# Harshs27/uGLAD

Hardware: AMD Instinct MI355X
Metric: GLAD unroll-steps/sec (batch D×D Θ-updates), M=1024 D=128 L=30 (higher is better)
Workload: dtype f32; 1 GPU; multi-task M=1024/GPU D=128 L=30 fp32 (BASELINE config 3; global batch 1024); pass=training step: forward + loss + backward + gradient exchange + Adam, sqrt_mode=ns10, parallelism=batch-sharded x1

## Files before the change

uglad_amd/csrc/cell_bwd.h:

```cpp
template <int NT>
__global__ __launch_bounds__(kThreads) void UGLAD_CELL_BWD_NAME(
    const float* __restrict__ Gnext, const float* __restrict__ S, const float* __restrict__ Zin,
    const float* __restrict__ half, const float* __restrict__ U, const float* __restrict__ beta,
    const float* __restrict__ lam_ptr, const float* __restrict__ params, float* __restrict__ Gout,
    float* __restrict__ grad_rho_partial, float* __restrict__ glam_partial, float* __restrict__ gws, int D, int mode,
#if UGLAD_CELL_BWD_GS
    int gs, int k_count, int lam_stride, float* __restrict__ gS) {
#else
    int gs, int k_count, int lam_stride) {
#endif
  constexpr int DP = NT * 32, LD = DP + 1;
  UGLAD_BIG_BUFFERS(sX, DP * LD, sY, DP * LD, gws)
  __shared__ float s_beta[DP], s_r[DP];
  __shared__ __attribute__((aligned(16))) float s_a0[DP], s_aN[DP];
  __shared__ float s_red[8];
  __shared__ float s_g[kWaves][kNRho + 1];
  const int tid = threadIdx.x, lane = tid & 63, w = tid >> 6;
  const size_t base = (size_t)blockIdx.x * D * D;
  const float* Sm = S + base;
  const float* Gm = Gnext + base;
  float* Go = Gout + base;
  const int grp = blockIdx.x / gs;
  params += (size_t)grp * kNParam;
  const size_t step_mdd = (size_t)gridDim.x * D * D, step_md = (size_t)gridDim.x * D;
  constexpr bool kPackA = NT <= 7;
  float g[kNRho];
  [[maybe_unused]] v2f g2[kNRho];
#pragma unroll
  for (int q = 0; q < kNRho; ++q) g[q] = 0.f, g2[q] = splat2(0.f);
  constexpr int kMaxQ = ((DP / 2) * (DP + 1) + kThreads - 1) / kThreads;
  constexpr bool kPre = DP <= 128;
  constexpr int kQ = kPre ? kMaxQ : 8;
  constexpr int kIShift = kPre ? 8 : 16, kJMask = (1 << kIShift) - 1;
  const int D1 = D + 1, total = ((D + 1) / 2) * D1;
  const int sp = kThreads / D1, sc = kThreads - sp * D1;
  auto entry = [&](int e, int p, int c) -> int {
    if (e >= total) return -1;
    if (c < D - p) return (p << kIShift) | (p + c);
    const int i = D - 1 - p;
    return (i == p) ? -1 : ((i << kIShift) | (i + (c - (D - p))));
  };
  auto advance = [&](int& p, int& c) {
    c += sc;
    p += sp;
    if (c >= D1) {
      c -= D1;
      ++p;
    }
  };
  __shared__ unsigned short s_ent[kPre ? kMaxQ : 1][kPre ? kThreads : 1];
  if constexpr (kPre) {
    int p = tid / D1, c = tid - p * D1;
    for (int q = 0; q < kMaxQ; ++q) {
      s_ent[q][tid] = (unsigned short)entry(tid + kThreads * q, p, c);
      advance(p, c);
    }
  }
#pragma unroll 1
  for (int s = 0; s < k_count; ++s) {
    const bool first = (s == 0), last = (s == k_count - 1);
    const int tid = opaque_v(threadIdx.x), lane = tid & 63;
    const int w = __builtin_amdgcn_readfirstlane(tid >> 6);
    const float* Zm = Zin + base - s * step_mdd;
    const float* Hm = half + base - s * step_mdd;
    const float* Um = U + base - s * step_mdd;
    const float* bm = beta + (size_t)blockIdx.x * D - s * step_md;
    const float lam = lam_ptr[(long)grp - (long)s * lam_stride];
    const float c4 = 4.0f / lam, inv_lam2 = 1.0f / (lam * lam);

    KSTAMP(0);
    constexpr int kV4 = DP * DP / 4, kC4 = DP / 4;
    constexpr bool kFull4 = kV4 % (8 * kThreads) == 0, kFull1 = (DP * DP) % (8 * kThreads) == 0;
    const bool vec16 = (D == DP) && (((reinterpret_cast<size_t>(U) | (first ? reinterpret_cast<size_t>(Gnext) : 0)) & 15) == 0);
    if (vec16) {
      if (first) {
        for (int v0 = 0; v0 < kV4; v0 += 8 * kThreads) {
          f4 u[8], gv[8];
#pragma unroll
          for (int q = 0; q < 8; ++q) {
            const int idx = v0 + q * kThreads + tid;
            const unsigned at = (kFull4 || idx < kV4) ? 16u * idx : 0u;
            u[q] = load_at<f4>(Um, at);
            gv[q] = load_at<f4>(Gm, at);
          }
#pragma unroll
          for (int q = 0; q < 8; ++q) {
            const int idx = v0 + q * kThreads + tid;
            if (kFull4 || idx < kV4) {
              const int i = idx / kC4, k = 4 * (idx - i * kC4);
              sX[i * LD + k] = u[q].x, sX[i * LD + k + 1] = u[q].y, sX[i * LD + k + 2] = u[q].z, sX[i * LD + k + 3] = u[q].w;
              sY[i * LD + k] = gv[q].x, sY[i * LD + k + 1] = gv[q].y, sY[i * LD + k + 2] = gv[q].z, sY[i * LD + k + 3] = gv[q].w;
            }
          }
        }
      } else {
        for (int v0 = 0; v0 < kV4; v0 += 8 * kThreads) {
          f4 u[8];
#pragma unroll
          for (int q = 0; q < 8; ++q) {
            const int idx = v0 + q * kThreads + tid;
            u[q] = load_at<f4>(Um, (kFull4 || idx < kV4) ? 16u * idx : 0u);
          }
#pragma unroll
          for (int q = 0; q < 8; ++q) {
            const int idx = v0 + q * kThreads + tid;
            if (kFull4 || idx < kV4) {
              const int i = idx / kC4, k = 4 * (idx - i * kC4);
              sX[i * LD + k] = u[q].x, sX[i * LD + k + 1] = u[q].y, sX[i * LD + k + 2] = u[q].z, sX[i * LD + k + 3] = u[q].w;
            }
          }
        }
      }
    } else {
      constexpr int si = kThreads / DP, sk = kThreads - si * DP;
      int i = tid / DP, k = tid - i * DP;
      int off = i * D + k;
      const int soff = si * D + sk, wrap = D - DP;
      if (first) {
        for (int idx0 = 0; idx0 < DP * DP; idx0 += 8 * kThreads) {
          float u[8], gv[8];
          int dst[8];
          bool in[8];
#pragma unroll
          for (int q = 0; q < 8; ++q) {
            in[q] = (kFull1 || idx0 + q * kThreads + tid < DP * DP) && i < D && k < D;
            const unsigned at = in[q] ? 4u * off : 0u;
            u[q] = load_at<float>(Um, at);
            gv[q] = load_at<float>(Gm, at);
            dst[q] = i * LD + k;
            i += si, k += sk, off += soff;
            if (k >= DP) k -= DP, ++i, off += wrap;
          }
          __builtin_amdgcn_sched_barrier(0);
#pragma unroll
          for (int q = 0; q < 8; ++q) {
            if (kFull1 || idx0 + q * kThreads + tid < DP * DP) {
              sX[dst[q]] = in[q] ? u[q] : 0.f;
              sY[dst[q]] = in[q] ? gv[q] : 0.f;
            }
          }
        }
      } else {
        for (int idx0 = 0; idx0 < DP * DP; idx0 += 8 * kThreads) {
          float u[8];
          int dst[8];
          bool in[8];
#pragma unroll
          for (int q = 0; q < 8; ++q) {
            in[q] = (kFull1 || idx0 + q * kThreads + tid < DP * DP) && i < D && k < D;
            u[q] = load_at<float>(Um, in[q] ? 4u * off : 0u);
            dst[q] = i * LD + k;
            i += si, k += sk, off += soff;
            if (k >= DP) k -= DP, ++i, off += wrap;
          }
          __builtin_amdgcn_sched_barrier(0);
#pragma unroll
          for (int q = 0; q < 8; ++q) {
            if (kFull1 || idx0 + q * kThreads + tid < DP * DP) sX[dst[q]] = in[q] ? u[q] : 0.f;
          }
        }
      }
    }
    const float be_ld = load_at<float>(bm, (tid < D) ? 4u * (unsigned)tid : 0u);
    [[maybe_unused]] float hx_a[kQ], zz_a[kQ], sv_a[kQ];
    if constexpr (kPre) {
      int ea[kQ];
#pragma unroll
      for (int u = 0; u < kQ; ++u) ea[u] = (int)(short)s_ent[u][tid];
#pragma unroll
      for (int u = 0; u < kQ; ++u) {
        const unsigned at = (unsigned)opaque_v((ea[u] >= 0) ? 4 * ((ea[u] >> kIShift) * D + (ea[u] & kJMask)) : 0);
        hx_a[u] = load_at<float>(Hm, at);
        zz_a[u] = load_at<float>(Zm, at);
        sv_a[u] = load_at<float>(Sm, at);
      }
    }
    float a2 = 0.f;
    if (tid < D) {
      const float be = be_ld;
      const float al = fmaf(be, be, c4);
      a2 = al * al;
    }
    const float nrmA = sqrtf(block_sum(a2, s_red));
    float r2 = 0.f;
    if (tid < DP) {
      float be = 0.f, r = 1.f;
      if (tid < D) {
        be = be_ld;
        r = sqrt_spectrum(be, c4, nrmA, mode);
        r2 = r * r;
      }
      s_beta[tid] = be;
      s_r[tid] = r;
    }
    const float nrmR = sqrtf(block_sum(r2, s_red));
    if (mode == UGLAD_SQRT_NS10 && tid < DP) {
      float a = s_r[tid] / nrmR;
      s_a0[tid] = a;
#pragma unroll
      for (int it = 0; it < kNsIters; ++it) a = 0.5f * a * (3.f - a * a);
      s_aN[tid] = a;
    }
    __syncthreads();

    KSTAMP(1);
    using TU = Tiles<NT, true>;
    [[maybe_unused]] const int p0 = tid / D1, c0 = tid - p0 * D1;
    float gz[kQ];
    {
      [[maybe_unused]] int p = p0, c = c0;
      for (int q0 = 0; q0 < kMaxQ; q0 += kQ) {
        int pk[kQ];
        float hx[kQ], zz[kQ], gn[kQ], sv[kQ];
        if constexpr (kPre) {
#pragma unroll
          for (int u = 0; u < kQ; ++u) pk[u] = (int)(short)s_ent[u][tid];
          float gt[kQ];
#pragma unroll
          for (int u = 0; u < kQ; ++u) {
            const int i = pk[u] >> kIShift, j = pk[u] & kJMask;
            const bool in = pk[u] >= 0;
            gn[u] = sY[opaque_v(in ? i * LD + j : 0)];
            gt[u] = sY[opaque_v(in ? j * LD + i : 0)];
          }
          static_assert(kPackA || !kPre, "the tabled entries go with the packed backward");
#pragma unroll
          for (int u = 0; u < kQ; ++u) {
            const int i = pk[u] >> kIShift, j = pk[u] & kJMask;
            hx[u] = hx_a[u], zz[u] = zz_a[u], sv[u] = sv_a[u];
            gn[u] = (i == j) ? gn[u] : 0.5f * (gn[u] + gt[u]);
          }
        } else {
#pragma unroll
          for (int u = 0; u < kQ; ++u) {
            pk[u] = (q0 + u < kMaxQ) ? entry(tid + kThreads * (q0 + u), p, c) : -1;
            advance(p, c);
            const int i = pk[u] >> kIShift, j = pk[u] & kJMask;
            const bool in = pk[u] >= 0;
            hx[u] = in ? Hm[i * D + j] : 0.f;
            zz[u] = in ? Zm[i * D + j] : 0.f;
            sv[u] = in ? Sm[i * D + j] : 0.f;
            gn[u] = in ? ((i == j) ? sY[i * LD + j] : 0.5f * (sY[i * LD + j] + sY[j * LD + i])) : 0.f;
          }
        }
        constexpr int kQ2 = (kQ + 1) / 2;
        if constexpr (kPackA) {
          [[maybe_unused]] const int tid_a = opaque_v(tid);
#pragma unroll
          for (int h = 0; h < kQ2; ++h) {
            const int u0 = 2 * h, u1 = (2 * h + 1 < kQ) ? 2 * h + 1 : 2 * h;
            const bool has1 = 2 * h + 1 < kQ;
            const int e0 = kPre ? (int)(short)s_ent[kPre ? u0 : 0][kPre ? tid_a : 0] : pk[u0];
            const int e1 = kPre ? (int)(short)s_ent[kPre ? u1 : 0][kPre ? tid_a : 0] : pk[u1];
            const bool in0 = e0 >= 0, in1 = has1 && e1 >= 0;
            const int i0 = e0 >> kIShift, j0 = e0 & kJMask, i1 = e1 >> kIShift, j1 = e1 & kJMask;
            const v2f x = {hx[u0], has1 ? hx[u1] : 0.f}, s2 = {sv[u0], has1 ? sv[u1] : 0.f}, z2 = {zz[u0], has1 ? zz[u1] : 0.f};
            const v2f gn2 = {gn[u0], has1 ? gn[u1] : 0.f};
            RhoAct2 act2;
            rho_forward2(params, x, s2, z2, act2);
            const bool on0 = in0 && fabsf(x.x) > act2.rho.x, on1 = in1 && fabsf(x.y) > act2.rho.y;
            const v2f gact = {on0 ? gn2.x : 0.f, on1 ? gn2.y : 0.f};
            const v2f g_rho = {on0 ? ((x.x > 0.f) ? -gn2.x : gn2.x) : 0.f, on1 ? ((x.y > 0.f) ? -gn2.y : gn2.y) : 0.f};
            const v2f wgt = {on0 ? ((i0 == j0) ? 1.f : 2.f) : 0.f, on1 ? ((i1 == j1) ? 1.f : 2.f) : 0.f};
            v2f gx1, gx3;
            rho_backward2(params, x, s2, z2, act2, g_rho, wgt, g2, gx1, gx3);
#pragma unroll
            for (int q = 0; q < kNRho; ++q) g2[q] = opaque_f2(g2[q]);
            gx3 = opaque_f2(gx3);
#if UGLAD_CELL_BWD_GS
            if (in0) gS[base + i0 * D + j0] += rho_backward_col(params, act2.half(0), g_rho.x, 1);
            if (in1) gS[base + i1 * D + j1] += rho_backward_col(params, act2.half(1), g_rho.y, 1);
#endif
            const v2f gh = gact + gx1;
            sY[opaque_v(in0 ? i0 * LD + j0 : DP)] = gh.x;
            sY[opaque_v(in0 ? j0 * LD + i0 : DP)] = gh.x;
            if (has1) {
              sY[opaque_v(in1 ? i1 * LD + j1 : DP)] = gh.y;
              sY[opaque_v(in1 ? j1 * LD + i1 : DP)] = gh.y;
            }
            if constexpr (kPre) {
              gz[u0] = gx3.x;
              if (has1) gz[u1] = gx3.y;
            } else {
              if (in0) Go[i0 * D + j0] = gx3.x;
              if (in1) Go[i1 * D + j1] = gx3.y;
            }
          }
        } else {
#pragma unroll
        for (int h = 0; h < kQ2; ++h) {
          const int u0 = 2 * h, u1 = (2 * h + 1 < kQ) ? 2 * h + 1 : 2 * h;
          const bool has1 = 2 * h + 1 < kQ;
          if (!has1 && pk[u0] < 0) continue;
          RhoAct2 act2;
          rho_forward2(params, (v2f){hx[u0], has1 ? hx[u1] : 0.f}, (v2f){sv[u0], has1 ? sv[u1] : 0.f},
                       (v2f){zz[u0], has1 ? zz[u1] : 0.f}, act2);
#pragma unroll
          for (int c2 = 0; c2 < 2; ++c2) {
            const int u = c2 ? u1 : u0;
            if ((c2 == 0 || has1) && pk[u] >= 0) {
              const int i = pk[u] >> kIShift, j = pk[u] & kJMask;
              const RhoAct act = act2.half(c2);
              const float x = hx[u];
              const bool active = fabsf(x) > act.rho;
              const float sgn = (x > 0.f) ? 1.f : ((x < 0.f) ? -1.f : 0.f);
              const float g_rho = active ? -sgn * gn[u] : 0.f;
              float gx1, gx3;
              rho_backward(params, x, sv[u], zz[u], act, g_rho, (i == j) ? 1.f : 2.f, g, gx1, gx3);
#if UGLAD_CELL_BWD_GS
              gS[base + i * D + j] += rho_backward_col(params, act, g_rho, 1);
#endif
              const float gh = (active ? gn[u] : 0.f) + gx1;
              sY[i * LD + j] = gh;
              sY[j * LD + i] = gh;
              if (kPre) gz[u] = gx3;
              else Go[i * D + j] = gx3;
            }
          }
        }
        }
      }
    }
    __syncthreads();

    KSTAMP(2);
    using T = Tiles<NT, false>;
    {
      f32x16 acc[T::kPerWave];
      gemm_lds<NT, false, false, false>(sY, sX, acc);
      __syncthreads();
      store_tiles<NT>(sY, acc);
    }
    __syncthreads();
    KSTAMP(3);
    float glam = 0.f;
    {
      f32x16 acc[TU::kPerWave];
      gemm_lds<NT, true, false, true>(sX, sY, acc);
      __syncthreads();
      KSTAMP(4);
#pragma unroll
      for (int n = 0; n < TU::kPerWave; ++n) {
        const int t = w + kWaves * n;
        if (t < TU::kCount) {
          int I, J;
          TU::ij(t, I, J);
          const int j = J * 32 + (lane & 31);
          const float a0j = s_a0[j], aNj = s_aN[j];
          const float rj = s_r[j], bj = s_beta[j];
          const float inv_2nrmR = 1.0f / (2.f * nrmR);
#pragma unroll
          for (int e4 = 0; e4 < 4; ++e4) {
            const int i0 = I * 32 + 8 * e4 + 4 * (lane >> 5);
            float Kr[4];
            if (mode == UGLAD_SQRT_EXACT) {
#pragma unroll
              for (int r = 0; r < 4; ++r) Kr[r] = 1.0f / (s_r[i0 + r] + rj);
            } else {
              const f4 a0 = *reinterpret_cast<const f4*>(&s_a0[i0]);
              const f4 aN = *reinterpret_cast<const f4*>(&s_aN[i0]);
              Kr[0] = ns_divided_difference(a0.x, a0j, aN.x, aNj, inv_2nrmR);
              Kr[1] = ns_divided_difference(a0.y, a0j, aN.y, aNj, inv_2nrmR);
              Kr[2] = ns_divided_difference(a0.z, a0j, aN.z, aNj, inv_2nrmR);
              Kr[3] = ns_divided_difference(a0.w, a0j, aN.w, aNj, inv_2nrmR);
            }
#pragma unroll
            for (int r = 0; r < 4; ++r) {
              const int e = 4 * e4 + r, i = i0 + r;
              if (I < J || i <= j) {
                float v = 0.f;
                if (i < D && j < D) {
                  const float K = Kr[r];
                  const float cij = acc[n][e];
                  if (i == j) glam = fmaf(cij, -2.f * K * inv_lam2, glam);
                  v = cij * 0.5f * fmaf(s_beta[i] + bj, K, -1.f);
                }
                sY[i * LD + j] = v;
                sY[j * LD + i] = v;
              }
            }
          }
        }
      }
    }
    __syncthreads();
    KSTAMP(5);
    {
      f32x16 acc[T::kPerWave];
      gemm_lds<NT, false, false, false>(sX, sY, acc);
      __syncthreads();
      store_tiles<NT>(sY, acc);
    }
    __syncthreads();
    KSTAMP(6);
    {
      f32x16 acc[TU::kPerWave];
      gemm_lds<NT, false, true, true>(sY, sX, acc);
      KSTAMP(7);
      __syncthreads();
#pragma unroll
      for (int n = 0; n < TU::kPerWave; ++n) {
        const int t = w + kWaves * n;
        if (t < TU::kCount) {
          int I, J;
          TU::ij(t, I, J);
#pragma unroll
          for (int e = 0; e < 16; ++e) sY[(I * 32 + acc_row(e, lane)) * LD + J * 32 + (lane & 31)] = acc[n][e];
        }
      }
    }
    __syncthreads();
    KSTAMP(20);
    {
      [[maybe_unused]] int p = p0, c = c0;
      for (int q0 = 0; q0 < kMaxQ; q0 += kQ) {
        int pk[kQ];
        float gb[kQ], sij[kQ];
#pragma unroll
        for (int u = 0; u < kQ; ++u) {
          if constexpr (kPre) {
            pk[u] = (int)(short)s_ent[u][tid];
          } else {
            pk[u] = (q0 + u < kMaxQ) ? entry(tid + kThreads * (q0 + u), p, c) : -1;
            advance(p, c);
          }
          const bool in = pk[u] >= 0;
          const int i = pk[u] >> kIShift, j = pk[u] & kJMask;
          gb[u] = sY[in ? i * LD + j : 0];
          sij[u] = load_at<float>(Sm, in ? 4u * ((unsigned)i * (unsigned)D + (unsigned)j) : 0u);
        }
        if (kPre) {
#pragma unroll
          for (int u = 0; u < kQ; ++u) {
            const bool in = pk[u] >= 0;
            const int i = pk[u] >> kIShift, j = pk[u] & kJMask;
            const float o = gz[u] - gb[u];
            sY[in ? i * LD + j : DP] = o;
            sY[in ? j * LD + i : DP] = o;
            glam = fmaf(in ? -sij[u] * inv_lam2 * ((i == j) ? 1.f : 2.f) : 0.f, gb[u], glam);
          }
        } else {
#pragma unroll
          for (int u = 0; u < kQ; ++u) {
            if (pk[u] >= 0) {
              const int i = pk[u] >> kIShift, j = pk[u] & kJMask;
              const float o = Go[i * D + j] - gb[u];
              sY[i * LD + j] = o;
              sY[j * LD + i] = o;
              glam = fmaf(-sij[u] * inv_lam2 * ((i == j) ? 1.f : 2.f), gb[u], glam);
            }
          }
        }
#if UGLAD_CELL_BWD_GS
        {
          const float inv_lam = 1.0f / lam;
#pragma unroll
          for (int u = 0; u < kQ; ++u) {
            if (pk[u] >= 0) {
              const int i = pk[u] >> kIShift, j = pk[u] & kJMask;
              const float v = fmaf(gb[u], inv_lam, gS[base + i * D + j]);
              gS[base + i * D + j] = v;
              gS[base + j * D + i] = v;
            }
          }
        }
#endif
      }
    }
    __syncthreads();
    KSTAMP(21);
    if (last) {
      const int si = kThreads / D, sj = kThreads - si * D;
      int i = tid / D, j = tid - i * D;
      for (int idx = tid; idx < D * D; idx += kThreads) {
        Go[idx] = sY[i * LD + j];
        j += sj;
        i += si;
        if (j >= D) {
          j -= D;
          ++i;
        }
      }
    }
    KSTAMP(8);
    if (last) {
#pragma unroll
      for (int q = 0; q < kNRho; ++q) {
        if constexpr (kPackA) g[q] = g2[q].x + g2[q].y;
        const float v = wave_sum(g[q]);
        if (lane == 0) s_g[w][q] = v;
      }
    }
    {
      const float v = wave_sum(glam);
      if (lane == 0) s_g[w][kNRho] = v;
    }
    __syncthreads();
    if (tid == kNRho || (last && tid < kNRho)) {
      float v = 0.f;
#pragma unroll
      for (int ww = 0; ww < kWaves; ++ww) v += s_g[ww][tid];
      if (tid < kNRho)
        grad_rho_partial[(size_t)blockIdx.x * kNRho + tid] += v;
      else
        (glam_partial - (size_t)s * gridDim.x)[blockIdx.x] = v;
    }
    KSTAMP(9);
  }
}
```

uglad_amd/csrc/glad_device.h:

```cpp
#pragma once
#include <hip/hip_runtime.h>

namespace uglad {

#ifndef UGLAD_THREADS
#define UGLAD_THREADS 512
#endif
constexpr int kThreads = UGLAD_THREADS;
constexpr int kWaves = kThreads / 64;
constexpr int kNsIters = 10;

constexpr int P_T = 0, P_RW1 = 1, P_RB1 = 10, P_RW2 = 13, P_RB2 = 22, P_RW3 = 25, P_RB3 = 28;
constexpr int P_LW1 = 29, P_LB1 = 35, P_LW2 = 38, P_LB2 = 41;
constexpr int kNParam = 42, kNRho = 28;

typedef float f32x16 __attribute__((ext_vector_type(16)));
struct alignas(16) f4 {
  float x, y, z, w;
};

#ifdef UGLAD_SIMT_EMUL
#define UGLAD_WAVE_SYNC() simt::wave_sync_point()
#else
#define UGLAD_WAVE_SYNC() asm volatile("s_waitcnt vmcnt(0) lgkmcnt(0)" ::: "memory")
#endif

template <int CTRL, int ROW_MASK = 0xf, int BANK_MASK = 0xf>
__device__ __forceinline__ float dpp_move(float v) {
  return __int_as_float(__builtin_amdgcn_update_dpp(0, __float_as_int(v), CTRL, ROW_MASK, BANK_MASK, false));
}

__device__ __forceinline__ float lane_xor1(float v) { return dpp_move<0xb1>(v); }

__device__ __forceinline__ float sum_halves(float v) {
#ifdef UGLAD_SIMT_EMUL
  return v + __shfl_xor(v, 32);
#else
  const auto r = __builtin_amdgcn_permlane32_swap(__float_as_uint(v), __float_as_uint(v), false, false);
  return __uint_as_float(r[0]) + __uint_as_float(r[1]);
#endif
}

__device__ __forceinline__ int opaque_v(int v) {
#ifndef UGLAD_SIMT_EMUL
  asm volatile("" : "+v"(v));
#endif
  return v;
}

template <typename T>
__device__ __forceinline__ T load_at(const float* __restrict__ base, unsigned bytes) {
  return *reinterpret_cast<const T*>(reinterpret_cast<const char*>(base) + bytes);
}

__device__ __forceinline__ float opaque_f(float v) {
#ifndef UGLAD_SIMT_EMUL
  asm volatile("" : "+v"(v));
#endif
  return v;
}

__device__ __forceinline__ int lane_now() {
#ifdef UGLAD_SIMT_EMUL
  return threadIdx.x & 63;
#else
  int l;
  asm volatile("v_mbcnt_lo_u32_b32 %0, -1, 0\n\tv_mbcnt_hi_u32_b32 %0, -1, %0" : "=v"(l));
  return l;
#endif
}

__device__ __forceinline__ float bcast_lane(float v, int src) {
  return __int_as_float(__builtin_amdgcn_readlane(__float_as_int(v), src));
}

__device__ __forceinline__ float wave_sum(float v) {
  v += dpp_move<0xb1>(v);
  v += dpp_move<0x4e>(v);
  v += dpp_move<0x124>(v);
  v += dpp_move<0x128>(v);
  v += dpp_move<0x142, 0xa>(v);
  v += dpp_move<0x143, 0xc>(v);
  return __int_as_float(__builtin_amdgcn_readlane(__float_as_int(v), 63));
}

__device__ __forceinline__ float block_sum(float v, float* s_red) {
  v = wave_sum(v);
  const int lane = threadIdx.x & 63, w = threadIdx.x >> 6;
  if (lane == 0) s_red[w] = v;
  __syncthreads();
  float t = 0.f;
#pragma unroll
  for (int i = 0; i < kWaves; ++i) t += s_red[i];
  __syncthreads();
  return t;
}

__device__ __forceinline__ float exp_acc(float x) {
  const float t = x * 1.44269504f;
  float e = fmaf(x, 1.44269504f, -t);
  e = fmaf(x, 1.925963033e-8f, e);
  const float r = __builtin_amdgcn_exp2f(t);
  return fmaf(r, e * 0.69314718f, r);
}

__device__ __forceinline__ float div_acc(float a, float b) {
  float q = __builtin_amdgcn_rcpf(b);
  q = fmaf(q, fmaf(-b, q, 1.0f), q);
  return a * q;
}

__device__ __forceinline__ float sigmoidf_(float x) {
  const float t = exp_acc(-fabsf(x));
  const float s = div_acc(1.0f, 1.0f + t);
  return (x >= 0.f) ? s : 1.0f - s;
}

__device__ __forceinline__ float tanhf_(float x) {
  const float t = exp_acc(-2.0f * fabsf(x));
  return copysignf(div_acc(1.0f - t, 1.0f + t), x);
}

struct RhoAct {
  float h1[3], h2[3], rho;
};

__device__ __forceinline__ void rho_forward(const float* __restrict__ p, float x1, float x2, float x3, RhoAct& a) {
#pragma unroll
  for (int o = 0; o < 3; ++o)
    a.h1[o] = tanhf_(fmaf(p[P_RW1 + 3 * o], x1, fmaf(p[P_RW1 + 3 * o + 1], x2, fmaf(p[P_RW1 + 3 * o + 2], x3, p[P_RB1 + o]))));
#pragma unroll
  for (int o = 0; o < 3; ++o)
    a.h2[o] = tanhf_(fmaf(p[P_RW2 + 3 * o], a.h1[0], fmaf(p[P_RW2 + 3 * o + 1], a.h1[1], fmaf(p[P_RW2 + 3 * o + 2], a.h1[2], p[P_RB2 + o]))));
  a.rho = sigmoidf_(fmaf(p[P_RW3], a.h2[0], fmaf(p[P_RW3 + 1], a.h2[1], fmaf(p[P_RW3 + 2], a.h2[2], p[P_RB3]))));
}

typedef float v2f __attribute__((ext_vector_type(2)));
__device__ __forceinline__ v2f opaque_f2(v2f v) {
#ifndef UGLAD_SIMT_EMUL
  asm volatile("" : "+v"(v));
#endif
  return v;
}
__device__ __forceinline__ v2f fma2(v2f a, v2f b, v2f c) { return __builtin_elementwise_fma(a, b, c); }
__device__ __forceinline__ v2f splat2(float a) { return (v2f){a, a}; }
__device__ __forceinline__ v2f exp_acc2(v2f x) {
  const v2f t = x * 1.44269504f;
  v2f e = fma2(x, splat2(1.44269504f), -t);
  e = fma2(x, splat2(1.925963033e-8f), e);
  const v2f r = {__builtin_amdgcn_exp2f(t.x), __builtin_amdgcn_exp2f(t.y)};
  return fma2(r, e * 0.69314718f, r);
}
__device__ __forceinline__ v2f div_acc2(v2f a, v2f b) {
  v2f q = {__builtin_amdgcn_rcpf(b.x), __builtin_amdgcn_rcpf(b.y)};
  q = fma2(q, fma2(-b, q, splat2(1.0f)), q);
  return a * q;
}
__device__ __forceinline__ v2f tanh2(v2f x) {
  const v2f t = exp_acc2(-2.0f * __builtin_elementwise_abs(x));
  const v2f r = div_acc2(1.0f - t, 1.0f + t);
  return (v2f){copysignf(r.x, x.x), copysignf(r.y, x.y)};
}
__device__ __forceinline__ v2f sigmoid2(v2f x) {
  const v2f t = exp_acc2(-__builtin_elementwise_abs(x));
  const v2f s = div_acc2(splat2(1.0f), 1.0f + t);
  return (v2f){(x.x >= 0.f) ? s.x : 1.0f - s.x, (x.y >= 0.f) ? s.y : 1.0f - s.y};
}
struct RhoAct2 {
  v2f h1[3], h2[3], rho;
  __device__ __forceinline__ RhoAct half(int c) const {
    RhoAct a;
#pragma unroll
    for (int o = 0; o < 3; ++o) {
      a.h1[o] = c ? h1[o].y : h1[o].x;
      a.h2[o] = c ? h2[o].y : h2[o].x;
    }
    a.rho = c ? rho.y : rho.x;
    return a;
  }
};
__device__ __forceinline__ void rho_forward2(const float* __restrict__ p, v2f x1, v2f x2, v2f x3, RhoAct2& a) {
#pragma unroll
  for (int o = 0; o < 3; ++o)
    a.h1[o] = tanh2(fma2(splat2(p[P_RW1 + 3 * o]), x1,
                         fma2(splat2(p[P_RW1 + 3 * o + 1]), x2, fma2(splat2(p[P_RW1 + 3 * o + 2]), x3, splat2(p[P_RB1 + o])))));
#pragma unroll
  for (int o = 0; o < 3; ++o)
    a.h2[o] = tanh2(fma2(splat2(p[P_RW2 + 3 * o]), a.h1[0],
                         fma2(splat2(p[P_RW2 + 3 * o + 1]), a.h1[1], fma2(splat2(p[P_RW2 + 3 * o + 2]), a.h1[2], splat2(p[P_RB2 + o])))));
  a.rho = sigmoid2(fma2(splat2(p[P_RW3]), a.h2[0], fma2(splat2(p[P_RW3 + 1]), a.h2[1], fma2(splat2(p[P_RW3 + 2]), a.h2[2], splat2(p[P_RB3])))));
}

__device__ __forceinline__ float soft_threshold(float x, float rho) {
  const float m = fabsf(x) - rho;
  return m > 0.f ? copysignf(m, x) : 0.f;
}

__device__ __forceinline__ void rho_backward(const float* __restrict__ p, float x1, float x2, float x3, const RhoAct& a,
                                             float g_rho, float w, float* g, float& gx1, float& gx3) {
  const float go = g_rho * a.rho * (1.f - a.rho);
  const float gow = go * w;
  float ga2[3], ga1[3];
#pragma unroll
  for (int h = 0; h < 3; ++h) {
    g[(P_RW3 - 1) + h] += gow * a.h2[h];
    ga2[h] = go * p[P_RW3 + h] * (1.f - a.h2[h] * a.h2[h]);
  }
  g[P_RB3 - 1] += gow;
#pragma unroll
  for (int o = 0; o < 3; ++o) {
    const float t = ga2[o] * w;
#pragma unroll
    for (int h = 0; h < 3; ++h) g[(P_RW2 - 1) + 3 * o + h] += t * a.h1[h];
    g[(P_RB2 - 1) + o] += t;
  }
#pragma unroll
  for (int h = 0; h < 3; ++h) {
    const float s = ga2[0] * p[P_RW2 + h] + ga2[1] * p[P_RW2 + 3 + h] + ga2[2] * p[P_RW2 + 6 + h];
    ga1[h] = s * (1.f - a.h1[h] * a.h1[h]);
  }
#pragma unroll
  for (int o = 0; o < 3; ++o) {
    const float t = ga1[o] * w;
    g[(P_RW1 - 1) + 3 * o + 0] += t * x1;
    g[(P_RW1 - 1) + 3 * o + 1] += t * x2;
    g[(P_RW1 - 1) + 3 * o + 2] += t * x3;
    g[(P_RB1 - 1) + o] += t;
  }
  gx1 = ga1[0] * p[P_RW1 + 0] + ga1[1] * p[P_RW1 + 3] + ga1[2] * p[P_RW1 + 6];
  gx3 = ga1[0] * p[P_RW1 + 2] + ga1[1] * p[P_RW1 + 5] + ga1[2] * p[P_RW1 + 8];
}

__device__ __forceinline__ float rho_backward_col(const float* __restrict__ p, const RhoAct& a, float g_rho, int col) {
  const float go = g_rho * a.rho * (1.f - a.rho);
  float ga2[3], ga1[3];
#pragma unroll
  for (int h = 0; h < 3; ++h) ga2[h] = go * p[P_RW3 + h] * (1.f - a.h2[h] * a.h2[h]);
#pragma unroll
  for (int h = 0; h < 3; ++h) {
    const float s = ga2[0] * p[P_RW2 + h] + ga2[1] * p[P_RW2 + 3 + h] + ga2[2] * p[P_RW2 + 6 + h];
    ga1[h] = s * (1.f - a.h1[h] * a.h1[h]);
  }
  return ga1[0] * p[P_RW1 + col] + ga1[1] * p[P_RW1 + 3 + col] + ga1[2] * p[P_RW1 + 6 + col];
}

__device__ __forceinline__ void rho_backward2(const float* __restrict__ p, v2f x1, v2f x2, v2f x3, const RhoAct2& a, v2f g_rho,
                                              v2f w, v2f* g2, v2f& gx1, v2f& gx3) {
  const v2f go = g_rho * a.rho * (1.f - a.rho);
  const v2f gow = go * w;
  v2f ga2[3], ga1[3];
#pragma unroll
  for (int h = 0; h < 3; ++h) {
    g2[(P_RW3 - 1) + h] = fma2(gow, a.h2[h], g2[(P_RW3 - 1) + h]);
    ga2[h] = go * p[P_RW3 + h] * (1.f - a.h2[h] * a.h2[h]);
  }
  g2[P_RB3 - 1] += gow;
#pragma unroll
  for (int o = 0; o < 3; ++o) {
    const v2f t = ga2[o] * w;
#pragma unroll
    for (int h = 0; h < 3; ++h) g2[(P_RW2 - 1) + 3 * o + h] = fma2(t, a.h1[h], g2[(P_RW2 - 1) + 3 * o + h]);
    g2[(P_RB2 - 1) + o] += t;
  }
#pragma unroll
  for (int h = 0; h < 3; ++h) {
    const v2f s = (h == 0) ? fma2(ga2[2], splat2(p[P_RW2 + 6]), fma2(ga2[0], splat2(p[P_RW2]), ga2[1] * p[P_RW2 + 3]))
                           : fma2(ga2[2], splat2(p[P_RW2 + 6 + h]), fma2(ga2[1], splat2(p[P_RW2 + 3 + h]), ga2[0] * p[P_RW2 + h]));
    ga1[h] = s * (1.f - a.h1[h] * a.h1[h]);
  }
#pragma unroll
  for (int o = 0; o < 3; ++o) {
    const v2f t = ga1[o] * w;
    g2[(P_RW1 - 1) + 3 * o + 0] = fma2(t, x1, g2[(P_RW1 - 1) + 3 * o + 0]);
    g2[(P_RW1 - 1) + 3 * o + 1] = fma2(t, x2, g2[(P_RW1 - 1) + 3 * o + 1]);
    g2[(P_RW1 - 1) + 3 * o + 2] = fma2(t, x3, g2[(P_RW1 - 1) + 3 * o + 2]);
    g2[(P_RB1 - 1) + o] += t;
  }
  gx1 = fma2(ga1[2], splat2(p[P_RW1 + 6]), fma2(ga1[0], splat2(p[P_RW1 + 0]), ga1[1] * p[P_RW1 + 3]));
  gx3 = opaque_f2(ga1[2] * p[P_RW1 + 8]) + fma2(ga1[1], splat2(p[P_RW1 + 5]), ga1[0] * p[P_RW1 + 2]);
}

__device__ __forceinline__ float lambda_forward(const float* __restrict__ p, float n, float lam_prev) {
  float o = p[P_LB2];
#pragma unroll
  for (int h = 0; h < 3; ++h)
    o = fmaf(p[P_LW2 + h], tanhf(fmaf(p[P_LW1 + 2 * h], n, fmaf(p[P_LW1 + 2 * h + 1], lam_prev, p[P_LB1 + h]))), o);
  return sigmoidf_(o);
}

__device__ __forceinline__ float sqrt_spectrum(float beta, float c, float nrmA, int mode) {
  const float alpha = fmaf(beta, beta, c);
  if (mode == 0) return sqrtf(alpha);
  float y = alpha / nrmA, z = 1.f;
#pragma unroll
  for (int it = 0; it < kNsIters; ++it) {
    const float T = 0.5f * (3.f - z * y);
    y = y * T;
    z = T * z;
  }
  return y * sqrtf(nrmA);
}

__device__ __forceinline__ float ns_divided_difference(float a0_i, float a0_j, float aN_i, float aN_j, float inv_2nrmR) {
  return div_acc(aN_i + aN_j, a0_i + a0_j) * inv_2nrmR;
}

__device__ __forceinline__ float shifted_spectrum(float be, int D, float lam, int mode, double* __restrict__ s3, float& alpha,
                                                  float& cond) {
  const int tid = threadIdx.x;
  const double c4 = 4.0 / (double)lam, b = (double)be;
  const double al = b * b + c4;
  const double r_exact = sqrt(al);
  if (tid < D) {
    s3[tid] = al * al;
    s3[D + tid] = 0.5 * (r_exact - b) * b;
    s3[2 * D + tid] = b * b;
  }
  __syncthreads();
  double* part = s3 + 3 * D;
  if ((tid >> 6) == 0) {
    const double* a = s3 + ((tid >> 4) < 3 ? (tid >> 4) : 2) * D;
    double s = 0.0, mx = 0.0, mn = 1e300;
    for (int i = tid & 15; i < D; i += 16) {
      const double v = a[i];
      s += v;
      mx = v > mx ? v : mx;
      mn = v < mn ? v : mn;
    }
#pragma unroll
    for (int o = 1; o < 16; o *= 2) {
      s += __shfl_xor(s, o);
      const double mxo = __shfl_xor(mx, o), mno = __shfl_xor(mn, o);
      mx = mxo > mx ? mxo : mx;
      mn = mno < mn ? mno : mn;
    }
    if ((tid & 15) == 0 && tid < 48) part[tid >> 4] = s;
    if (tid == 32) {
      part[3] = mx;
      part[4] = mn;
    }
  }
  __syncthreads();
  const double n2 = part[0], pb = part[1], bb = part[2], b2max = part[3], b2min = part[4];
  cond = (float)((b2max + c4) / (b2min + c4));
  double a_opt = (bb > 0.0) ? -pb / bb : 0.0;
  a_opt = a_opt < 0.0 ? 0.0 : (a_opt > 1.0 ? 1.0 : a_opt);
  alpha = (float)a_opt;
  double r = r_exact;
  if (mode != 0) {
    const double nrmA = sqrt(n2);
    double y = al / nrmA, z = 1.0;
#pragma unroll
    for (int it = 0; it < kNsIters; ++it) {
      const double T = 0.5 * (3.0 - z * y);
      y = y * T;
      z = T * z;
    }
    r = y * sqrt(nrmA);
  }
  const double psi = 0.5 * (r - b) + (double)alpha * b;
  __syncthreads();
  return (tid < D) ? (float)psi : 0.f;
}

template <int DP>
__device__ __forceinline__ void pair_of(int r, int k, int& i1, int& i2) {
  constexpr int m = DP - 1;
  if (k == 0) {
    i1 = m;
    i2 = r;
  } else {
    i1 = r + k;
    if (i1 >= m) i1 -= m;
    i2 = r + m - k;
    if (i2 >= m) i2 -= m;
  }
}

template <int DP>
__device__ void jacobi_eig(float* __restrict__ A, float* __restrict__ V, float* s_t, float* s_s, float* s_h, float* s_red,
                           int* s_flag) {
  constexpr int LD = DP + 1, H = DP / 2;
  const int tid = threadIdx.x;
  float fro = 0.f;
  for (int idx = tid; idx < DP * DP; idx += kThreads) {
    const float v = A[(idx / DP) * LD + (idx % DP)];
    fro = fmaf(v, v, fro);
  }
  fro = sqrtf(block_sum(fro, s_red));
  const float thresh = 1e-8f * fro;
  for (int sweep = 0; sweep < 16; ++sweep) {
    if (tid == 0) *s_flag = 0;
    __syncthreads();
    for (int r = 0; r < DP - 1; ++r) {
      if (tid < H) {
        int p, q;
        pair_of<DP>(r, tid, p, q);
        const float apq = A[p * LD + q];
        float t = 0.f, s = 0.f, h = 0.f;
        if (fabsf(apq) > thresh) {
          const float app = A[p * LD + p], aqq = A[q * LD + q];
          const float tau = (aqq - app) / (2.f * apq);
          t = copysignf(1.f, tau) / (fabsf(tau) + sqrtf(fmaf(tau, tau, 1.f)));
          const float c = 1.f / sqrtf(fmaf(t, t, 1.f));
          s = t * c;
          h = s / (1.f + c);
          *s_flag = 1;
        }
        s_t[tid] = t;
        s_s[tid] = s;
        s_h[tid] = h;
      }
      __syncthreads();
      for (int b = tid; b < H * H; b += kThreads) {
        const int kr = b / H, kc = b - kr * H;
        int r1, r2, c1, c2;
        pair_of<DP>(r, kr, r1, r2);
        pair_of<DP>(r, kc, c1, c2);
        const float x11 = A[r1 * LD + c1], x12 = A[r1 * LD + c2], x21 = A[r2 * LD + c1], x22 = A[r2 * LD + c2];
        float z11, z12, z21, z22;
        if (kr == kc) {
          const float t = s_t[kr];
          z11 = x11 - t * x12;
          z22 = x22 + t * x12;
          z12 = (t != 0.f) ? 0.f : x12;
          z21 = (t != 0.f) ? 0.f : x21;
        } else {
          const float sr = s_s[kr], hr = s_h[kr], sc = s_s[kc], hc = s_h[kc];
          const float y11 = x11 - sr * (x21 + hr * x11), y21 = x21 + sr * (x11 - hr * x21);
          const float y12 = x12 - sr * (x22 + hr * x12), y22 = x22 + sr * (x12 - hr * x22);
          z11 = y11 - sc * (y12 + hc * y11);
          z12 = y12 + sc * (y11 - hc * y12);
          z21 = y21 - sc * (y22 + hc * y21);
          z22 = y22 + sc * (y21 - hc * y22);
        }
        A[r1 * LD + c1] = z11;
        A[r1 * LD + c2] = z12;
        A[r2 * LD + c1] = z21;
        A[r2 * LD + c2] = z22;
      }
      for (int b = tid; b < DP * H; b += kThreads) {
        const int i = b / H, kc = b - i * H;
        int c1, c2;
        pair_of<DP>(r, kc, c1, c2);
        const float sc = s_s[kc], hc = s_h[kc];
        const float v1 = V[i * LD + c1], v2 = V[i * LD + c2];
        V[i * LD + c1] = v1 - sc * (v2 + hc * v1);
        V[i * LD + c2] = v2 + sc * (v1 - hc * v2);
      }
      __syncthreads();
    }
    if (*s_flag == 0) break;
    __syncthreads();
  }
  __syncthreads();
}

template <int NT, bool UPPER>
struct Tiles {
  static constexpr int kCount = UPPER ? NT * (NT + 1) / 2 : NT * NT;
  static constexpr int kPerWave = (kCount + kWaves - 1) / kWaves;
  __device__ static __forceinline__ void ij(int t, int& I, int& J) {
    if (UPPER) {
      int i = 0, rem = t;
      while (rem >= NT - i) {
        rem -= NT - i;
        ++i;
      }
      I = i;
      J = i + rem;
    } else {
      I = t / NT;
      J = t - I * NT;
    }
  }
};

__device__ __forceinline__ int acc_row(int reg, int lane) { return (reg & 3) + 8 * (reg >> 2) + 4 * (lane >> 5); }

__device__ __forceinline__ void mfma_tile(const float* __restrict__ Ap, int a_si, int a_sk, const float* __restrict__ Bp,
                                          int b_sk, int b_sj, int K, f32x16& acc) {
  const int lane = opaque_v(threadIdx.x) & 63, li = lane & 31, kh = lane >> 5;
  const float* a = Ap + li * a_si + kh * a_sk;
  const float* b = Bp + li * b_sj + kh * b_sk;
  float a0[8], b0[8], a1[8], b1[8];
#pragma unroll
  for (int u = 0; u < 8; ++u) {
    a0[u] = a[2 * u * a_sk];
    b0[u] = b[2 * u * b_sk];
  }
  for (int k = 0; k < K; k += 16) {
    const bool more = k + 16 < K;
    const float* an = a + (more ? 16 * a_sk : 0);
    const float* bn = b + (more ? 16 * b_sk : 0);
#pragma unroll
    for (int u = 0; u < 8; ++u) {
      a1[u] = an[2 * u * a_sk];
      b1[u] = bn[2 * u * b_sk];
    }
#pragma unroll
    for (int u = 0; u < 8; ++u) acc = __builtin_amdgcn_mfma_f32_32x32x2f32(a0[u], b0[u], acc, 0, 0, 0);
#pragma unroll
    for (int u = 0; u < 8; ++u) {
      a0[u] = a1[u];
      b0[u] = b1[u];
    }
    a = an;
    b = bn;
  }
}

#if defined(UGLAD_BF16X3) && !defined(UGLAD_SIMT_EMUL)
#include "../../scripts/retired/bf16x3_tile.h"
#define UGLAD_GEMM_TILE mfma_tile_bf16x3
#else
#define UGLAD_GEMM_TILE mfma_tile
#endif

template <int NT, bool TA, bool TB, bool UPPER>
__device__ __forceinline__ void gemm_lds(const float* __restrict__ X, const float* __restrict__ Y,
                                         f32x16 (&acc)[Tiles<NT, UPPER>::kPerWave]) {
  constexpr int DP = NT * 32, LD = DP + 1;
  using T = Tiles<NT, UPPER>;
  const int w = __builtin_amdgcn_readfirstlane(opaque_v(threadIdx.x) >> 6);
#pragma unroll
  for (int n = 0; n < T::kPerWave; ++n) {
    const int t = w + kWaves * n;
#pragma unroll
    for (int e = 0; e < 16; ++e) acc[n][e] = 0.f;
    if (t < T::kCount) {
      int I, J;
      T::ij(t, I, J);
      UGLAD_GEMM_TILE(TA ? X + I * 32 : X + I * 32 * LD, TA ? 1 : LD, TA ? LD : 1, TB ? Y + J * 32 * LD : Y + J * 32,
                      TB ? 1 : LD, TB ? LD : 1, DP, acc[n]);
    }
  }
}

template <int NT>
__device__ __forceinline__ void store_tiles(float* __restrict__ Y, const f32x16 (&acc)[Tiles<NT, false>::kPerWave]) {
  constexpr int LD = NT * 32 + 1;
  using T = Tiles<NT, false>;
  const int tid = opaque_v(threadIdx.x), lane = tid & 63, w = __builtin_amdgcn_readfirstlane(tid >> 6);
#pragma unroll
  for (int n = 0; n < T::kPerWave; ++n) {
    const int t = w + kWaves * n;
    if (t < T::kCount) {
      int I, J;
      T::ij(t, I, J);
#pragma unroll
      for (int e = 0; e < 16; ++e) Y[(I * 32 + acc_row(e, lane)) * LD + J * 32 + (lane & 31)] = acc[n][e];
    }
  }
}

#ifdef UGLAD_STAMPS
__device__ unsigned long long g_cwg[4096][3];
__device__ unsigned long long g_lstamps[4][96];
__device__ unsigned long long g_kstamps[32];
#define KSTAMP(i) do { if (threadIdx.x == 0 && blockIdx.x == 0) g_kstamps[i] = __builtin_amdgcn_s_memtime(); } while (0)
#define UGLAD_STAMP(ws, i) do { if (threadIdx.x == 0 && (i) < 64) (ws).stamp[i] = __builtin_amdgcn_s_memtime(); } while (0)
#elif defined(UGLAD_PHASE_EXIT)
__device__ int g_exit_at;
#define KSTAMP(i) do { if (g_exit_at == 100 + (i)) __builtin_amdgcn_endpgm(); } while (0)
#define UGLAD_STAMP(ws, i) do { if (g_exit_at == (i)) __builtin_amdgcn_endpgm(); } while (0)
#else
#define KSTAMP(i) do {} while (0)
#define UGLAD_STAMP(ws, i) do {} while (0)
#endif

__device__ __forceinline__ void copy_out_matrix(float* __restrict__ dst, const float* __restrict__ src, int D, int LD) {
  const int tid = threadIdx.x;
  if (((D & 3) == 0) && ((reinterpret_cast<size_t>(dst) & 15) == 0)) {
    const int D4 = D >> 2;
    for (int idx = tid; idx < D * D4; idx += kThreads) {
      const int i = idx / D4, j = 4 * (idx - i * D4);
      const float* p = src + i * LD + j;
      f4 v = {p[0], p[1], p[2], p[3]};
      *reinterpret_cast<f4*>(dst + (size_t)i * D + j) = v;
    }
  } else {
    const int si = kThreads / D, sj = kThreads - si * D;
    int i = tid / D, j = tid - i * D;
    for (int idx = tid; idx < D * D; idx += kThreads) {
      dst[idx] = src[i * LD + j];
      j += sj;
      i += si;
      if (j >= D) {
        j -= D;
        ++i;
      }
    }
  }
}

template <int DP>
constexpr int kTfacFloats = (DP / 32) * 1024;
template <int DP>
constexpr int kWsPerMatrix = 3 * DP + kTfacFloats<DP>;
template <int DP>
constexpr int big_floats() {
  return 2 * ((DP * (DP + 1) + 3) & ~3);
}
#define UGLAD_BIG_BUFFERS(A, NA, B, NB, GWS)                                                                     \
  constexpr bool kGM = DP > 128;                                                                                 \
  __shared__ __attribute__((aligned(16))) float A##_lds[kGM ? 4 : (NA)];                                         \
  __shared__ __attribute__((aligned(16))) float B##_lds[kGM ? 4 : (NB)];                                         \
  float* A = kGM ? (GWS) + (size_t)gridDim.x * kWsPerMatrix<DP> + (size_t)blockIdx.x * big_floats<DP>() : A##_lds; \
  float* B = kGM ? A + big_floats<DP>() / 2 : B##_lds;

template <int DP>
__device__ __forceinline__ float* tfac_behind_flags(float* ws, int M, int m) {
  static_assert(kTfacFloats<DP> / 2 >= 4, "flags and packed T factors outgrow the T region: M + 3 <= M kTfacFloats / 2 needs kTfacFloats / 2 >= 4");
  return ws + (size_t)M * 3 * DP + ((M + 3) & ~3) + (size_t)m * (kTfacFloats<DP> / 2);
}

}
```

Measured before the change: 1.326 million unroll-steps/s.

## Split leftover upper-triangular GEMM tiles across two waves with K-split and LDS reduction

For D=128 (NT=4) the upper-triangular tile set has more tiles than waves, so a few waves ran a second full 32x32 tile while the others sat idle. This splits each extra tile's K dimension in half across two waves. Each wave writes its partial accumulator half to a shared-memory scratch buffer, and each then finishes half of the tile's rows. The aim is to balance load across waves in the two symmetric backward GEMMs, at the cost of extra LDS traffic, a scratch buffer, and more complex epilogue indexing.

Result: no change. 1.338 million unroll-steps/s (median of 6 runs) (+1.0%).

```diff
diff --git a/uglad_amd/csrc/cell_bwd.h b/uglad_amd/csrc/cell_bwd.h
--- a/uglad_amd/csrc/cell_bwd.h
+++ b/uglad_amd/csrc/cell_bwd.h
@@ -205,6 +205,7 @@
 
     KSTAMP(1);
     using TU = Tiles<NT, true>;
+    using SU = SplitUpper<NT>;
     [[maybe_unused]] const int p0 = tid / D1, c0 = tid - p0 * D1;
     float gz[kQ];
     {
@@ -336,12 +337,15 @@
     float glam = 0.f;
     {
       f32x16 acc[TU::kPerWave];
-      gemm_lds<NT, true, false, true>(sX, sY, acc);
+      if constexpr (SU::kOn) SU::template product<true, false>(sX, sY, acc);
+      else gemm_lds<NT, true, false, true>(sX, sY, acc);
       __syncthreads();
+      if constexpr (SU::kOn) SU::finish(acc);
       KSTAMP(4);
 #pragma unroll
       for (int n = 0; n < TU::kPerWave; ++n) {
-        const int t = w + kWaves * n;
+        const int t = (SU::kOn && n == 1) ? SU::tile1(w) : w + kWaves * n;
+        [[maybe_unused]] const int rofs = (SU::kOn && n == 1) ? SU::rofs1(w) : 0;
         if (t < TU::kCount) {
           int I, J;
           TU::ij(t, I, J);
@@ -351,7 +355,10 @@
           const float inv_2nrmR = 1.0f / (2.f * nrmR);
 #pragma unroll
           for (int e4 = 0; e4 < 4; ++e4) {
-            const int i0 = I * 32 + 8 * e4 + 4 * (lane >> 5);
+            if constexpr (SU::kOn) {
+              if (n == 1 && e4 >= 2) continue;
+            }
+            const int i0 = SU::kOn ? I * 32 + 8 * e4 + 4 * (lane >> 5) + rofs : I * 32 + 8 * e4 + 4 * (lane >> 5);
             float Kr[4];
             if (mode == UGLAD_SQRT_EXACT) {
 #pragma unroll
@@ -395,15 +402,24 @@
     KSTAMP(6);
     {
       f32x16 acc[TU::kPerWave];
-      gemm_lds<NT, false, true, true>(sY, sX, acc);
+      if constexpr (SU::kOn) SU::template product<false, true>(sY, sX, acc);
+      else gemm_lds<NT, false, true, true>(sY, sX, acc);
       KSTAMP(7);
       __syncthreads();
+      if constexpr (SU::kOn) SU::finish(acc);
 #pragma unroll
       for (int n = 0; n < TU::kPerWave; ++n) {
-        const int t = w + kWaves * n;
+        const int t = (SU::kOn && n == 1) ? SU::tile1(w) : w + kWaves * n;
         if (t < TU::kCount) {
           int I, J;
           TU::ij(t, I, J);
+          if constexpr (SU::kOn) {
+            if (n == 1) {
+#pragma unroll
+              for (int e = 0; e < 8; ++e) sY[(I * 32 + acc_row(e, lane) + SU::rofs1(w)) * LD + J * 32 + (lane & 31)] = acc[n][e];
+              continue;
+            }
+          }
 #pragma unroll
           for (int e = 0; e < 16; ++e) sY[(I * 32 + acc_row(e, lane)) * LD + J * 32 + (lane & 31)] = acc[n][e];
         }
diff --git a/uglad_amd/csrc/glad_device.h b/uglad_amd/csrc/glad_device.h
--- a/uglad_amd/csrc/glad_device.h
+++ b/uglad_amd/csrc/glad_device.h
@@ -554,6 +554,60 @@
   }
 }
 
+#ifndef UGLAD_SPLIT_UPPER
+#define UGLAD_SPLIT_UPPER 1
+#endif
+template <int NT>
+struct SplitUpper {
+  using T = Tiles<NT, true>;
+  static constexpr int kExtra = T::kCount - kWaves;
+  static constexpr bool kOn = UGLAD_SPLIT_UPPER && NT * 32 <= 128 && kExtra > 0 && 2 * kExtra <= 4 && T::kPerWave == 2;
+  static constexpr int kPartFloats = 2 * kExtra * 8 * 64;
+  __device__ static __forceinline__ float* part() {
+    __shared__ float s_part[kPartFloats];
+    return s_part;
+  }
+  __device__ static __forceinline__ int tile1(int w) { return (w < 2 * kExtra) ? kWaves + ((w < kExtra) ? w : w - kExtra) : T::kCount; }
+  __device__ static __forceinline__ int rofs1(int w) { return (w < kExtra) ? 0 : 16; }
+  template <bool TA, bool TB>
+  __device__ static __forceinline__ void product(const float* __restrict__ X, const float* __restrict__ Y, f32x16 (&acc)[2]) {
+    constexpr int DP = NT * 32, LD = DP + 1;
+    const int tid = opaque_v(threadIdx.x), lane = tid & 63, w = __builtin_amdgcn_readfirstlane(tid >> 6);
+#pragma unroll
+    for (int n = 0; n < 2; ++n)
+#pragma unroll
+      for (int e = 0; e < 16; ++e) acc[n][e] = 0.f;
+    {
+      int I, J;
+      T::ij(w, I, J);
+      UGLAD_GEMM_TILE(TA ? X + I * 32 : X + I * 32 * LD, TA ? 1 : LD, TA ? LD : 1, TB ? Y + J * 32 * LD : Y + J * 32, TB ? 1 : LD,
+                      TB ? LD : 1, DP, acc[0]);
+    }
+    if (w < 2 * kExtra) {
+      int I, J;
+      T::ij(tile1(w), I, J);
+      const bool owner = w < kExtra;
+      const int k0 = owner ? 0 : DP / 2;
+      const float* A = (TA ? X + I * 32 : X + I * 32 * LD) + k0 * (TA ? LD : 1);
+      const float* B = (TB ? Y + J * 32 * LD : Y + J * 32) + k0 * (TB ? 1 : LD);
+      UGLAD_GEMM_TILE(A, TA ? 1 : LD, TA ? LD : 1, B, TB ? 1 : LD, TB ? LD : 1, DP / 2, acc[1]);
+      float* mine = part() + w * 512 + lane;
+#pragma unroll
+      for (int r = 0; r < 8; ++r) mine[64 * r] = owner ? opaque_f(acc[1][8 + r]) : opaque_f(acc[1][r]);
+    }
+  }
+  __device__ static __forceinline__ void finish(f32x16 (&acc)[2]) {
+    const int tid = opaque_v(threadIdx.x), lane = tid & 63, w = __builtin_amdgcn_readfirstlane(tid >> 6);
+    if (w < 2 * kExtra) {
+      const bool owner = w < kExtra;
+      const float* theirs = part() + (owner ? w + kExtra : w - kExtra) * 512 + lane;
+#pragma unroll
+      for (int r = 0; r < 8; ++r)
+        acc[1][r] = (owner ? opaque_f(acc[1][r]) : opaque_f(acc[1][8 + r])) + theirs[64 * r];
+    }
+  }
+};
+
 #ifdef UGLAD_STAMPS
 __device__ unsigned long long g_cwg[4096][3];
 __device__ unsigned long long g_lstamps[4][96];
```
